# jerry102102102/RL_brain_trainer

Measured on AMD Instinct MI355X. Metric: env-steps/sec (whole node), Stage-5 Approach->Finisher PPO loops (rollout + update); value = the Approach loop, finisher.value = the Finisher loop, higher is better.
Workload: dtype f32

## Files before the change

### rl_brain_trainer_amd/csrc/kp1_mlp.hip

```cpp
#include <hip/hip_runtime.h>
#include <hip/hip_ext.h>

#include <cmath>
#include <cstddef>
#include <cstdlib>
#include <cstring>
#include <vector>

#include "../../include/kp1_ppo.h"
#include "kp1_device.hpp"
#include "kp1_host.hpp"

using kp1::fail;
using namespace kp1;

typedef float f32x16 __attribute__((ext_vector_type(16)));
typedef float f32x4 __attribute__((ext_vector_type(4)));

namespace {

constexpr int ACT = KP1_MLP_ACT, HEADS = 8;
constexpr float LOG_SQRT_2PI = 0.9189385332046727f;

enum { EPI_BIAS_TANH = 0, EPI_DTANH = 1 };
// ... 981 lines not shown

constexpr int ADAM_BLOCK = 256, VEC = 1;
template <bool POP = false>
__global__ void __launch_bounds__(ADAM_BLOCK) adam_kernel(float* __restrict__ p, float* __restrict__ g, float* __restrict__ m, float* __restrict__ v,
                                                   int64_t n, const double* __restrict__ partials, int n_partials, float lr, float eps, float max_norm,
                                                   float bc1, float bc2_sqrt, const ParamLayout L, const Packed k_, int zero_grad,
                                                   const int* __restrict__ step_counter, int host_step, const int* __restrict__ actor_extra,
                                                   unsigned r_partials, const float* __restrict__ hparams) {
  __shared__ float scale_s;
  const Packed k = POP ? packed_replica(k_, L, blockIdx.y) : k_;
  if constexpr (POP) {
    const unsigned o = blockIdx.y * (unsigned)n;
    p += o; g += o; m += o; v += o;
    partials += blockIdx.y * r_partials;
    if (hparams) {
      const float* e = hparams + blockIdx.y * (unsigned)HP_FIELDS;
      lr = e[HP_LR];
      eps = e[HP_EPS];
      max_norm = e[HP_MAX_NORM];
    }
  }
  const int64_t i0 = ((int64_t)blockIdx.x * ADAM_BLOCK + threadIdx.x) * VEC;
  float g_in[VEC], m_in[VEC], v_in[VEC], p_in[VEC];
#pragma unroll
  for (int j = 0; j < VEC; ++j) {
    const int64_t il = i0 + j < n ? i0 + j : n - 1;
    g_in[j] = g[il]; m_in[j] = m[il]; v_in[j] = v[il]; p_in[j] = p[il];
  }
  const int extra = *actor_extra;
  float base_step = (float)host_step;
  if (step_counter) base_step = (float)*step_counter;
  double s = 0.0;
  if (threadIdx.x < 64) {
    for (int q = threadIdx.x; q < n_partials; q += 64) s += partials[q];
    for (int off = 32; off > 0; off >>= 1) s += __shfl_xor(s, off);
  }
  if (threadIdx.x == 0) {
    const float norm = (float)sqrt(s);
    scale_s = max_norm > 0.f ? fminf(max_norm / (norm + 1e-6f), 1.f) : 1.f;
  }
  if (step_counter) {
    bc1 = 1.f - powf(0.9f, base_step);
    bc2_sqrt = sqrtf(1.f - powf(0.999f, base_step));
  }
  float bc1_a = bc1, bc2_sqrt_a = bc2_sqrt;
  if (extra != 0) {
    const float st = base_step + (float)extra;
    bc1_a = 1.f - powf(0.9f, st);
    bc2_sqrt_a = sqrtf(1.f - powf(0.999f, st));
  }
  __syncthreads();
  const float scale = scale_s;
  float pn[VEC], mn[VEC], vn[VEC];
#pragma unroll
  for (int j = 0; j < VEC; ++j) {
    const int64_t i = i0 + j;
    const bool actor = extra != 0 && ((i >= L.p_w1 && i < L.v_w1) || (i >= L.a_w && i < L.c_w));
    const float b1 = actor ? bc1_a : bc1, b2 = actor ? bc2_sqrt_a : bc2_sqrt;
    const float gi = g_in[j] * scale;
    mn[j] = 0.9f * m_in[j] + 0.1f * gi;
    vn[j] = 0.999f * v_in[j] + 0.001f * gi * gi;
    const float denom = sqrtf(vn[j]) / b2 + eps;
    pn[j] = p_in[j] - (lr / b1) * (mn[j] / denom);
  }
#pragma unroll
  for (int j = 0; j < VEC; ++j) {
    const int64_t i = i0 + j;
// ... 193 lines not shown
    const float pn = p_in - sh[1] * (mn / denom);
    m[i] = mn; v[i] = vn; p[i] = pn;
    pack_one(i, pn, L, k);
  }
}

__global__ void anchor_count_kernel(int* __restrict__ actor_extra) { *actor_extra += 1; }

#include "kp1_env_step.inc"
#include "kp1_eval_step.inc"
#include "kp1_mlp_tile.inc"
#include "kp1_mlp_fused.inc"

}

struct kp1_mlp {
  int device = 0, H = 0, Hp = 0, max_batch = 0;
  int K = 1;
  ParamLayout L;
  Packed k{};
  float* h1 = nullptr;
  float* h2 = nullptr;
  float* dz2 = nullptr;
  float* dz1 = nullptr;
  float* xf = nullptr;
  int bf16x3 = 0;
  unsigned short* sp_h1 = nullptr; unsigned short* sp_dz2 = nullptr; unsigned short* sp_dz1 = nullptr; unsigned short* sp_xf = nullptr;
  double* partials = nullptr;
  double* anchor_partials = nullptr;
  float* slab = nullptr;
  float* slab1 = nullptr;
  float* bslab = nullptr;
  float* hpart = nullptr;
  int n_finalize_blocks = 0;
  int* step_dev = nullptr;
  float* hparams_dev = nullptr;
  bool hparams_on = false;
  int last_s2_n = 0, last_s1_n = 0;
  int fused = 1;
  const float* last_params = nullptr;
  bool slab_stale = false;
  std::vector<void*> allocs;
  int profile = 0;
  struct ProfPair { hipEvent_t a, b; };
  std::vector<ProfPair> prof[KP1_MLP_PROFILE_SLOTS];
  int prof_used[KP1_MLP_PROFILE_SLOTS] = {0, 0, 0, 0};
};

namespace {
struct ProfSlotInFlight { hipEvent_t a = nullptr, b = nullptr; bool attached = false; };
thread_local ProfSlotInFlight tl_prof;

struct ProfScope {
  kp1_mlp* m; int slot; hipStream_t stream; bool on;
  ProfScope(kp1_mlp* m_, int slot_, hipStream_t s_) : m(m_), slot(slot_), stream(s_), on(m_->profile != 0) {
    if (!on) return;
    auto& v = m->prof[slot];
    if (m->prof_used[slot] >= (int)v.size()) {
      kp1_mlp::ProfPair p{};
      if (hipEventCreate(&p.a) != hipSuccess || hipEventCreate(&p.b) != hipSuccess) { on = false; return; }
      v.push_back(p);
    }
    tl_prof.a = v[m->prof_used[slot]].a;
    tl_prof.b = v[m->prof_used[slot]].b;
    tl_prof.attached = false;
  }
  ~ProfScope() {
    if (!on) return;
// ... 110 lines not shown
}

int launch_fused_infer_env(const FusedArgs& fa, int env_mode, hipStream_t stream) {
  const size_t bytes = sizeof(float) * FU_LDS_FLOATS;
  const dim3 grid((fa.n + FU_BM - 1) / FU_BM, 1, fa.value ? 2 : 1);
  if (env_mode == KP1_MODE_DOCK) {
    HIP_TRY(hipFuncSetAttribute((const void*)mlp_tile_kernel<false, 2, 2>, hipFuncAttributeMaxDynamicSharedMemorySize, (int)bytes));
    hipLaunchKernelGGL((mlp_tile_kernel<false, 2, 2>), grid, dim3(FU_NTH), bytes, stream, fa);
  } else {
    HIP_TRY(hipFuncSetAttribute((const void*)mlp_tile_kernel<false, 2, 1>, hipFuncAttributeMaxDynamicSharedMemorySize, (int)bytes));
    hipLaunchKernelGGL((mlp_tile_kernel<false, 2, 1>), grid, dim3(FU_NTH), bytes, stream, fa);
  }
  return KP1_OK;
}

int launch_fused_infer(const FusedArgs& fa, hipStream_t stream) {
  const size_t bytes = sizeof(float) * FU_LDS_FLOATS;
  const bool want_pi = fa.mean || fa.action || fa.clipped || fa.log_prob;
  if (!want_pi && !fa.value) return KP1_OK;
  FusedArgs f = fa;
  const bool both = want_pi && fa.value;
  if (!both) f.net_base = want_pi ? 0 : 1;
  const dim3 grid((fa.n + FU_BM - 1) / FU_BM, 1, both ? 2 : 1);
  if (fa.inp == 64) {
    HIP_TRY(hipFuncSetAttribute((const void*)mlp_tile_kernel<false, 2>, hipFuncAttributeMaxDynamicSharedMemorySize, (int)bytes));
    hipLaunchKernelGGL((mlp_tile_kernel<false, 2>), grid, dim3(FU_NTH), bytes, stream, f);
  } else {
    HIP_TRY(hipFuncSetAttribute((const void*)mlp_tile_kernel<false, 4>, hipFuncAttributeMaxDynamicSharedMemorySize, (int)bytes));
    hipLaunchKernelGGL((mlp_tile_kernel<false, 4>), grid, dim3(FU_NTH), bytes, stream, f);
  }
  return KP1_OK;
}

int launch_tn_frag(const TnFragArgs& t, hipStream_t stream) {
  if (t.n_chunks2 > 64 || t.n_chunks1 > 64) return fail(KP1_ERR_INVALID, "too many batch chunks for the partial-gradient slabs");
  const size_t bytes = sizeof(float) * TN_SPLIT_LDS_FLOATS;
  HIP_TRY(hipFuncSetAttribute((const void*)gemm_tn_split_kernel, hipFuncAttributeMaxDynamicSharedMemorySize, (int)bytes));
  KP1_LAUNCH(gemm_tn_split_kernel, dim3(32 * t.n_chunks2 + 16 * t.n_chunks1), dim3(256), bytes, stream, t);
  return KP1_OK;
}

int launch_forward_layers(kp1_mlp* m, const float* obs, int obs_stride, const int64_t* idx, int n, hipStream_t stream) {
  const int Hp = m->Hp, IN = m->L.IN, INP = m->L.INP;
  const int64_t act_stride = (int64_t)m->max_batch * Hp;
  GemmNT g{};
  g.reps = m->K;
  g.r_A = idx ? 0u : (unsigned)(n * obs_stride); g.r_gather = (unsigned)n;
  g.r_W = (unsigned)(2 * Hp * INP); g.r_bias = (unsigned)(2 * Hp); g.r_C = (unsigned)(2 * act_stride);
  g.A = obs; g.lda = obs_stride; g.strideA = 0; g.gather = idx;
  g.W = m->k.w1p; g.strideW = (int64_t)Hp * INP;
  g.bias = m->k.b1; g.strideBias = Hp;
  g.C = m->h1; g.ldc = Hp; g.strideC = act_stride;
  g.aux = nullptr; g.strideAux = 0; g.colsum = nullptr; g.strideColsum = 0;
  g.M = n; g.N = Hp; g.K = INP; g.Kreal = obs_stride >= INP ? INP : IN;
  int rc = launch_nt<EPI_BIAS_TANH>(g, stream);
  if (rc != KP1_OK) return rc;
  g.A = m->h1; g.lda = Hp; g.strideA = act_stride; g.gather = nullptr;
  g.r_A = (unsigned)(2 * act_stride); g.r_W = (unsigned)(2 * Hp * Hp);
  g.W = m->k.w2; g.strideW = (int64_t)Hp * Hp;
  g.bias = m->k.b2;
  g.C = m->h2;
  g.K = Hp; g.Kreal = Hp;
  rc = launch_nt<EPI_BIAS_TANH>(g, stream);
  if (rc != KP1_OK) return rc;
  HIP_TRY(kp1::launch_status());
  return KP1_OK;
}

}

namespace {
// ... 78 lines not shown
  m->H = hidden;
  m->L = make_layout(hidden, obs_dim);
  m->Hp = m->L.Hp;
  m->max_batch = (max_batch + 127) / 128 * 128;
  const int64_t Hp = m->Hp, mb = m->max_batch, INP = m->L.INP, K = m->K;
  auto alloc = [&](void** p, size_t bytes) -> int {
    if (hipMalloc(p, bytes) != hipSuccess) return fail(KP1_ERR_ALLOC, "hipMalloc failed in kp1_mlp_create");
    m->allocs.push_back(*p);
    return hipMemset(*p, 0, bytes) == hipSuccess ? KP1_OK : fail(KP1_ERR_NO_DEVICE, "hipMemset failed");
  };
  int rc = KP1_OK;
#define MLP_ALLOC(ptr, count) if (rc == KP1_OK) rc = alloc((void**)&(ptr), sizeof(*(ptr)) * (size_t)(count))
  MLP_ALLOC(m->k.w1p, K * 2 * Hp * INP);
  MLP_ALLOC(m->k.b1, K * 2 * Hp);
  MLP_ALLOC(m->k.w2, K * 2 * Hp * Hp);
  MLP_ALLOC(m->k.w2t, K * 2 * Hp * Hp);
  MLP_ALLOC(m->k.w1f, K * 2 * Hp * INP);
  MLP_ALLOC(m->k.w2f, K * 2 * Hp * Hp);
  MLP_ALLOC(m->k.w2tf, K * 2 * Hp * Hp);
  MLP_ALLOC(m->k.b2, K * 2 * Hp);
  MLP_ALLOC(m->k.w3, K * HEADS * Hp);
  MLP_ALLOC(m->k.b3, K * HEADS);
  MLP_ALLOC(m->k.log_std, K * HEADS);
  MLP_ALLOC(m->h1, K * 2 * mb * Hp);
  MLP_ALLOC(m->h2, K * 2 * mb * Hp);
  MLP_ALLOC(m->dz2, K * 2 * mb * Hp);
  MLP_ALLOC(m->dz1, K * 2 * mb * Hp);
  MLP_ALLOC(m->xf, mb * INP);
  MLP_ALLOC(m->partials, K * PARTIALS_STRIDE);
  if (Hp == 128) MLP_ALLOC(m->anchor_partials, K * ANCHOR_PARTIALS);
  MLP_ALLOC(m->slab, K * 64 * 2 * Hp * Hp);
  MLP_ALLOC(m->slab1, K * 64 * 2 * Hp * INP);
  MLP_ALLOC(m->step_dev, 4);
  if (K > 1) MLP_ALLOC(m->hparams_dev, K * HP_FIELDS);
  MLP_ALLOC(m->bslab, K * (mb / 32) * 2 * Hp);
  MLP_ALLOC(m->hpart, K * (mb / 32) * (10 * Hp + 32));
#undef MLP_ALLOC
  if (rc != KP1_OK) {
    kp1_mlp_destroy(m);
    return rc;
  }
  *out = m;
  return KP1_OK;
}
}

extern "C" {

int kp1_mlp_destroy(kp1_mlp* m) {
  if (!m) return KP1_OK;
  (void)hipSetDevice(m->device);
  (void)hipDeviceSynchronize();
  for (void* p : m->allocs) (void)hipFree(p);
  for (void* p : {(void*)m->sp_h1, (void*)m->sp_dz2, (void*)m->sp_dz1, (void*)m->sp_xf}) (void)hipFree(p);
  for (auto& v : m->prof)
    for (auto& pr : v) {
      (void)hipEventDestroy(pr.a);
      (void)hipEventDestroy(pr.b);
    }
  delete m;
  return KP1_OK;
}

int kp1_mlp_set_option(kp1_mlp* m, int32_t option, int32_t value) {
  if (!m) return fail(KP1_ERR_INVALID, "NULL argument");
  if (option == KP1_MLP_OPT_FUSED) {
// ... 249 lines not shown
    a.dz2 = m->dz2;
    a.hpart = m->hpart; a.hpart_stride = hpart_stride;
    a.r_act = (unsigned)(2 * act_stride); a.r_hpart = (unsigned)hpart_rep; a.r_partials = (unsigned)PARTIALS_STRIDE;
    a.hparams = pop && m->hparams_on ? m->hparams_dev : nullptr;
    {
      const dim3 hgrid((n + HEAD_ROWS - 1) / HEAD_ROWS, m->K);
      const size_t hbytes = sizeof(float) * (HEADS * Hp + HEAD_ROWS * 8 + 84 + 2 * HEAD_ROWS * (Hp + 4));
      if (pop) {
        HIP_TRY(hipFuncSetAttribute((const void*)head_train_kernel<128, true>, hipFuncAttributeMaxDynamicSharedMemorySize, (int)hbytes));
        hipLaunchKernelGGL((head_train_kernel<128, true>), hgrid, dim3(256), hbytes, stream, a);
      } else if (Hp == 256) {
        HIP_TRY(hipFuncSetAttribute((const void*)head_train_kernel<256>, hipFuncAttributeMaxDynamicSharedMemorySize, (int)hbytes));
        hipLaunchKernelGGL(head_train_kernel<256>, hgrid, dim3(256), hbytes, stream, a);
      } else {
        HIP_TRY(hipFuncSetAttribute((const void*)head_train_kernel<128>, hipFuncAttributeMaxDynamicSharedMemorySize, (int)hbytes));
        hipLaunchKernelGGL(head_train_kernel<128>, hgrid, dim3(256), hbytes, stream, a);
      }
    }
    GemmNT g{};
    g.A = m->dz2; g.lda = Hp; g.strideA = act_stride; g.gather = nullptr;
    g.W = m->k.w2t; g.strideW = (int64_t)Hp * Hp;
    g.bias = nullptr; g.strideBias = 0;
    g.C = m->dz1; g.ldc = Hp; g.strideC = act_stride;
    g.aux = m->h1; g.strideAux = act_stride;
    g.colsum = m->bslab; g.strideColsum = Hp;
    g.M = n; g.N = Hp; g.K = Hp; g.Kreal = Hp;
    g.reps = m->K;
    g.r_A = g.r_C = g.r_aux = (unsigned)(2 * act_stride); g.r_W = (unsigned)(2 * Hp * Hp);
    g.r_colsum = (unsigned)((m->max_batch / 32) * 2 * Hp);
    rc = launch_nt<EPI_DTANH>(g, stream);
    if (rc != KP1_OK) return rc;
  }

  int s2_n = 0, s1_n = 0;
  if (fused) {
    TnFragArgs t{};
    t.inp = INP;
    t.dz2 = m->dz2; t.h1 = m->h1; t.dz1 = m->dz1; t.act_stride = act_stride; t.xf = m->xf;
    t.slab2 = m->slab; t.s2_net = (int64_t)Hp * Hp; t.s2_chunk = 2 * t.s2_net;
    t.slab1 = m->slab1; t.s1_net = (int64_t)Hp * INP; t.s1_chunk = 2 * t.s1_net;
    t.groups = (n + FU_BM - 1) / FU_BM * (FU_BM / 8);
    auto up8 = [](int v) { return (v + 7) / 8 * 8; };
    t.cg2 = up8((t.groups + TN_SPLIT2 - 1) / TN_SPLIT2);
    t.cg1 = up8((t.groups + TN_SPLIT1 - 1) / TN_SPLIT1);
    t.n_chunks2 = (t.groups + t.cg2 - 1) / t.cg2;
    t.n_chunks1 = (t.groups + t.cg1 - 1) / t.cg1;
    if (m->bf16x3) {
      TnBf16Args b{};
      b.dz2 = m->sp_dz2; b.h1 = m->sp_h1; b.dz1 = m->sp_dz1; b.plane = (int64_t)2 * m->max_batch * Hp; b.net = (int64_t)m->max_batch * Hp;
      b.xf = m->sp_xf; b.plane_x = (int64_t)m->max_batch * INP; b.inp = INP;
      b.slab2 = t.slab2; b.s2_net = t.s2_net; b.s2_chunk = t.s2_chunk; b.slab1 = t.slab1; b.s1_net = t.s1_net; b.s1_chunk = t.s1_chunk;
      b.frags = t.groups / 2; b.cf2 = t.cg2 / 2; b.cf1 = t.cg1 / 2; b.n_chunks2 = t.n_chunks2; b.n_chunks1 = t.n_chunks1;
      const size_t bytes = sizeof(float) * TN_SPLIT_LDS_FLOATS;
      HIP_TRY(hipFuncSetAttribute((const void*)gemm_tn_bf16x3_kernel, hipFuncAttributeMaxDynamicSharedMemorySize, (int)bytes));
      ProfScope ps(m, KP1_MLP_PROFILE_WGRAD, stream);
      KP1_LAUNCH(gemm_tn_bf16x3_kernel, dim3(32 * b.n_chunks2 + 16 * b.n_chunks1), dim3(256), bytes, stream, b);
    } else {
      ProfScope ps(m, KP1_MLP_PROFILE_WGRAD, stream);
      rc = launch_tn_frag(t, stream);
    }
    if (rc != KP1_OK) return rc;
    s2_n = t.n_chunks2;
    s1_n = t.n_chunks1;
  } else {
    GemmTN t{};
    t.B = n;
    t.chunk = tn_chunk_rows(n, (Hp / 128) * (Hp / 128) * 2);
    t.D = m->dz2; t.ldd = Hp; t.strideD = act_stride;
    t.X = m->h1; t.ldx = Hp; t.strideX = act_stride; t.gatherX = nullptr;
    t.Nload = Hp; t.n_i_tiles = Hp / 128;
    rc = launch_tn(m, t, Hp / 128, Hp, m->slab, &s2_n, stream);
    if (rc != KP1_OK) return rc;
    t.D = m->dz1;
    t.X = obs; t.ldx = obs_stride; t.strideX = 0; t.gatherX = idx;
    t.Nload = obs_stride >= INP ? INP : IN; t.n_i_tiles = 1;
    t.chunk = tn_chunk_rows(n, (Hp / 128) * 2);
    rc = launch_tn(m, t, Hp / 128, INP, m->slab1, &s1_n, stream);
    if (rc != KP1_OK) return rc;
  }
  FinalizeArgs f{};
  f.L = L;
  f.slab2 = m->slab; f.s2_ld = Hp; f.s2_net = (int64_t)Hp * Hp; f.s2_chunk = 2 * f.s2_net; f.s2_n = s2_n;
  f.slab1 = m->slab1; f.s1_ld = INP; f.s1_net = (int64_t)Hp * INP; f.s1_chunk = 2 * f.s1_net; f.s1_n = s1_n;
  f.bslab = m->bslab; f.b_net = Hp; f.b_tile = 2 * Hp; f.b_n = fused ? (n + FU_BM - 1) / FU_BM * (FU_BM / 32) : nt_row_tiles(n, Hp);
  f.hpart = m->hpart; f.h_stride = 10 * Hp + 32; f.h_n = (n + HEAD_ROWS - 1) / HEAD_ROWS;
  f.ent_coef = ent_coef; f.inv_count = inv_count; f.log_std = m->k.log_std;
  f.grad = grad_out; f.stats = stats_out; f.sumsq = m->partials + 2 * N_PARTIALS;
  f.step_counter = m->step_dev;
  f.r_slab2 = (unsigned)(64 * f.s2_chunk); f.r_slab1 = (unsigned)(64 * f.s1_chunk); f.r_bslab = (unsigned)((m->max_batch / 32) * 2 * Hp);
  f.r_hpart = (unsigned)hpart_rep; f.r_sumsq = (unsigned)PARTIALS_STRIDE;
  f.hparams = pop && m->hparams_on ? m->hparams_dev : nullptr;
  const int n_main = (int)((finalize_vec_items(L) + 255) / 256);
  m->n_finalize_blocks = n_main + (int)((finalize_wide_count(L) + 3 + 31) / 32);
  if (m->n_finalize_blocks > 2048) return fail(KP1_ERR_INVALID, "parameter vector too large for the sum-of-squares partial buffer");
  {
    ProfScope ps(m, KP1_MLP_PROFILE_FINALIZE, stream);
    if (pop)
      KP1_LAUNCH(grad_finalize_kernel<true>, dim3(m->n_finalize_blocks, m->K), dim3(256), 0, stream, f, n_main);
    else
      KP1_LAUNCH(grad_finalize_kernel<false>, dim3(m->n_finalize_blocks), dim3(256), 0, stream, f, n_main);
  }
  HIP_TRY(kp1::launch_status());
  return KP1_OK;
}

int kp1_mlp_profile_read(kp1_mlp* m, float* out_us, int32_t* out_launches) {
  if (!m || !out_us || !out_launches) return fail(KP1_ERR_INVALID, "NULL argument to kp1_mlp_profile_read");
  int rc = mlp_check_device(m);
  if (rc != KP1_OK) return rc;
  for (int k = 0; k < KP1_MLP_PROFILE_SLOTS; ++k) {
    double total_ms = 0.0;
    for (int i = 0; i < m->prof_used[k]; ++i) {
      HIP_TRY(hipEventSynchronize(m->prof[k][i].b));
      float ms = 0.f;
      HIP_TRY(hipEventElapsedTime(&ms, m->prof[k][i].a, m->prof[k][i].b));
      total_ms += ms;
    }
    out_launches[k] = m->prof_used[k];
    out_us[k] = m->prof_used[k] > 0 ? (float)(total_ms * 1e3 / m->prof_used[k]) : 0.f;
    m->prof_used[k] = 0;
  }
  return KP1_OK;
}

int kp1_mlp_time_kernels(kp1_mlp* m, const float* obs, int32_t obs_stride, int32_t n, int32_t iters, float* out_ms, double* out_flops,
                         void* stream_) {
  if (!m || !obs || !out_ms || !out_flops || iters <= 0) return fail(KP1_ERR_INVALID, "bad argument to kp1_mlp_time_kernels");
  if (m->K > 1) return fail(KP1_ERR_UNSUPPORTED, "kp1_mlp_time_kernels is not available on population handles");
  if (n <= 0 || n > m->max_batch) return fail(KP1_ERR_INVALID, "n exceeds the workspace max_batch");
  int rc = mlp_check_device(m);
  if (rc != KP1_OK) return rc;
  hipStream_t stream = (hipStream_t)stream_;
  const int Hp = m->Hp, IN = m->L.IN, INP = m->L.INP;
// ... 9 lines not shown
    for (int it = 0; it < iters; ++it) {
      GemmNT g{};
      g.gather = nullptr; g.ldc = Hp; g.strideC = act_stride; g.M = n; g.N = Hp;
      if (which == 0) {
        g.A = m->h1; g.lda = Hp; g.strideA = act_stride; g.W = m->k.w2; g.strideW = (int64_t)Hp * Hp; g.bias = m->k.b2; g.strideBias = Hp;
        g.C = m->h2; g.K = Hp; g.Kreal = Hp;
        if (launch_nt<EPI_BIAS_TANH>(g, stream) != KP1_OK) return KP1_ERR_NO_DEVICE;
      } else if (which == 1) {
        g.A = m->dz2; g.lda = Hp; g.strideA = act_stride; g.W = m->k.w2t; g.strideW = (int64_t)Hp * Hp; g.C = m->dz1; g.aux = m->h1;
        g.strideAux = act_stride; g.K = Hp; g.Kreal = Hp;
        if (launch_nt<EPI_DTANH>(g, stream) != KP1_OK) return KP1_ERR_NO_DEVICE;
      } else if (which == 2) {
        GemmTN t{};
        t.B = n; t.chunk = tn_chunk_rows(n, (Hp / 128) * (Hp / 128) * 2);
        t.D = m->dz2; t.ldd = Hp; t.strideD = act_stride; t.X = m->h1; t.ldx = Hp; t.strideX = act_stride;
        t.Nload = Hp; t.n_i_tiles = Hp / 128;
        if (launch_tn(m, t, Hp / 128, Hp, m->slab, nullptr, stream) != KP1_OK) return KP1_ERR_NO_DEVICE;
      } else if (which == 3) {
        g.A = obs; g.lda = obs_stride; g.strideA = 0; g.W = m->k.w1p; g.strideW = (int64_t)Hp * INP; g.bias = m->k.b1; g.strideBias = Hp;
        g.C = m->h1; g.K = INP; g.Kreal = obs_stride >= INP ? INP : IN;
        if (launch_nt<EPI_BIAS_TANH>(g, stream) != KP1_OK) return KP1_ERR_NO_DEVICE;
      } else if (which == 4) {
        FusedArgs fa{};
        fa.obs = obs; fa.obs_stride = obs_stride; fa.Kreal = obs_stride >= INP ? INP : IN; fa.inp = INP; fa.idx = nullptr; fa.n = n;
        fa.k = m->k;
        fa.actions = m->h2; fa.old_logp = m->h2 + (int64_t)ACT * n; fa.adv = m->h2 + (int64_t)(ACT + 1) * n; fa.ret = m->h2 + (int64_t)(ACT + 2) * n;
        fa.adv_mode = 3; fa.adv_mean = 0.f; fa.adv_inv_std = 1.f;
        fa.clip_range = 0.2f; fa.vf_coef = 0.5f; fa.inv_count = 1.f / n;
        fa.h1 = m->h1; fa.dz2 = m->dz2; fa.dz1 = m->dz1; fa.act_stride = act_stride; fa.xf = m->xf;
        fa.bslab = m->bslab; fa.hpart = m->hpart; fa.hpart_stride = 10 * Hp + 32;
        if (launch_fused(fa, stream) != KP1_OK) return KP1_ERR_NO_DEVICE;
      } else {
        TnFragArgs t{};
    t.inp = INP;
        t.dz2 = m->dz2; t.h1 = m->h1; t.dz1 = m->dz1; t.act_stride = act_stride; t.xf = m->xf;
        t.slab2 = m->slab; t.s2_net = (int64_t)Hp * Hp; t.s2_chunk = 2 * t.s2_net;
        t.slab1 = m->slab1; t.s1_net = (int64_t)Hp * INP; t.s1_chunk = 2 * t.s1_net;
        t.groups = (n + FU_BM - 1) / FU_BM * (FU_BM / 8);
        t.cg2 = ((t.groups + TN_SPLIT2 - 1) / TN_SPLIT2 + 7) / 8 * 8;
        t.cg1 = ((t.groups + TN_SPLIT1 - 1) / TN_SPLIT1 + 7) / 8 * 8;
        t.n_chunks2 = (t.groups + t.cg2 - 1) / t.cg2;
        t.n_chunks1 = (t.groups + t.cg1 - 1) / t.cg1;
        if (launch_tn_frag(t, stream) != KP1_OK) return KP1_ERR_NO_DEVICE;
      }
    }
    HIP_TRY(hipEventRecord(e1, stream));
    HIP_TRY(hipEventSynchronize(e1));
    float ms = 0.f;
    HIP_TRY(hipEventElapsedTime(&ms, e0, e1));
    out_ms[which] = ms / iters;
    return KP1_OK;
  };
  for (int which : {3, 0, 1, 2}) {
    rc = time_it(which);
    if (rc != KP1_OK) return rc;
  }
  out_ms[4] = out_ms[5] = 0.f;
  out_flops[4] = out_flops[5] = 0.0;
  if (Hp == FU_HP) {
    for (int which : {4, 5}) {
      rc = time_it(which);
      if (rc != KP1_OK) return rc;
    }
  }
  const double M = n, H = Hp;
  out_flops[0] = 2.0 * 2.0 * M * H * H;
  out_flops[1] = 2.0 * 2.0 * M * H * H;
  out_flops[2] = 2.0 * 2.0 * M * H * H;
  out_flops[3] = 2.0 * 2.0 * M * H * INP;
  if (Hp == FU_HP) {
    out_flops[4] = 2.0 * 2.0 * M * (H * (double)INP + 2.0 * H * H);
    out_flops[5] = 2.0 * 2.0 * M * (H * H + H * (double)INP);
  }
  (void)hipEventDestroy(e0);
  (void)hipEventDestroy(e1);
  return KP1_OK;
// ... 53 lines not shown
    xcds += fresh ? 1 : 0;
  }
  out[0] = (int)total; out[1] = pairs; out[2] = same; out[3] = rr; out[4] = n_cus; out[5] = (int)seen.size(); out[6] = (int)host[total]; out[7] = xcds;
  return KP1_OK;
}

#ifdef KP1_CLK_TRACE
int kp1_debug_clk_trace(unsigned long long* out) {
  HIP_TRY(hipDeviceSynchronize());
  HIP_TRY(hipMemcpyFromSymbol(out, HIP_SYMBOL(kp1_clk_buf), sizeof(unsigned long long) * 2 * 1024 * 4));
  return KP1_OK;
}
#endif

#ifdef KP1_NT_TRACE
int kp1_debug_nt_trace(unsigned long long* out, int clear) {
  HIP_TRY(hipDeviceSynchronize());
  if (out) HIP_TRY(hipMemcpyFromSymbol(out, HIP_SYMBOL(kp1_nt_trace_buf), sizeof(unsigned long long) * KP1_TRACE_SLOTS * KP1_TRACE_WGS));
  if (clear) {
    std::vector<unsigned long long> z(KP1_TRACE_SLOTS * KP1_TRACE_WGS, 0ull);
    HIP_TRY(hipMemcpyToSymbol(HIP_SYMBOL(kp1_nt_trace_buf), z.data(), sizeof(unsigned long long) * z.size()));
  }
  return KP1_OK;
}
#endif

int kp1_mlp_adam_step(kp1_mlp* m, float* params, float* grad, float* exp_avg, float* exp_avg_sq, float lr, float eps, float max_grad_norm,
                      int32_t step, int32_t zero_grad, void* stream_) {
  if (!m || !params || !grad || !exp_avg || !exp_avg_sq) return fail(KP1_ERR_INVALID, "bad argument to kp1_mlp_adam_step");
  int rc = mlp_check_device(m);
  if (rc != KP1_OK) return rc;
  hipStream_t stream = (hipStream_t)stream_;
  const int64_t n = m->L.total;
  const bool fused_norm = (zero_grad & 2) && m->n_finalize_blocks > 0;
  const double* norm_partials = fused_norm ? m->partials + 2 * N_PARTIALS : m->partials + N_PARTIALS;
  const int n_norm_partials = fused_norm ? m->n_finalize_blocks : N_PARTIALS;
  ProfScope ps(m, KP1_MLP_PROFILE_ADAM, stream);
  const bool pop = m->K > 1;
  if (!fused_norm) {
    if (pop)
      hipLaunchKernelGGL(sumsq_partials_kernel<true>, dim3(N_PARTIALS, m->K), dim3(256), 0, stream, grad, n, m->partials + N_PARTIALS, (unsigned)PARTIALS_STRIDE);
    else
      hipLaunchKernelGGL(sumsq_partials_kernel<false>, dim3(N_PARTIALS), dim3(256), 0, stream, grad, n, m->partials + N_PARTIALS, 0u);
  }
  zero_grad = 0;
  const int host_step = step > 0 ? step : 1;
  const float bc1 = 1.f - std::pow(0.9f, (float)host_step);
  const float bc2 = 1.f - std::pow(0.999f, (float)host_step);
  Packed kfmt = m->k;
  const bool frag_only = m->fused && m->Hp == FU_HP;
  kfmt.formats = frag_only ? PACK_FRAG : (PACK_SLAB | PACK_FRAG);
  m->last_params = params;
  if (frag_only) m->slab_stale = true;
  const int* step_arg = step > 0 ? (const int*)nullptr : (const int*)m->step_dev;
  if (pop)
    KP1_LAUNCH(adam_kernel<true>, dim3((unsigned)((n + ADAM_BLOCK - 1) / ADAM_BLOCK), m->K), dim3(ADAM_BLOCK), 0, stream, params, grad, exp_avg, exp_avg_sq, n,
               norm_partials, n_norm_partials, lr, eps, max_grad_norm, bc1, std::sqrt(bc2), m->L, kfmt, zero_grad, step_arg, host_step,
               (const int*)m->step_dev + 1, (unsigned)PARTIALS_STRIDE, m->hparams_on ? (const float*)m->hparams_dev : (const float*)nullptr);
  else
    KP1_LAUNCH(adam_kernel<false>, dim3((unsigned)((n + ADAM_BLOCK - 1) / ADAM_BLOCK)), dim3(ADAM_BLOCK), 0, stream, params, grad, exp_avg, exp_avg_sq, n, norm_partials,
               n_norm_partials, lr, eps, max_grad_norm, bc1, std::sqrt(bc2), m->L, kfmt, zero_grad, step_arg, host_step, (const int*)m->step_dev + 1, 0u,
               (const float*)nullptr);
  HIP_TRY(kp1::launch_status());
  return KP1_OK;
}

int kp1_mlp_anchor_loss_grad(kp1_mlp* m, const float* obs, int32_t obs_stride, const int64_t* idx, int32_t n, const float* teacher_actions,
                             float loss_weight, float* grad_out, float* loss_out, void* stream_) {
  if (!m || !obs || !teacher_actions || !grad_out || !loss_out) return fail(KP1_ERR_INVALID, "NULL argument to kp1_mlp_anchor_loss_grad");
// ... 106 lines not shown
```

### rl_brain_trainer_amd/csrc/kp1_mlp_fused.inc

```

struct TnFragArgs {
  const float* dz2; const float* h1; const float* dz1; int64_t act_stride;
  const float* xf; int inp;
  float* slab2; int64_t s2_net, s2_chunk;
  float* slab1; int64_t s1_net, s1_chunk;
  int groups, cg2, n_chunks2, cg1, n_chunks1;
};

template <int RA, int CB>
__device__ __forceinline__ void tn_split_tile(const float* __restrict__ Af, int a_ncb, const float* __restrict__ Bf, int b_ncb, int g_begin, int g_end,
                                              float* __restrict__ out, int out_ld, float* lds) {
  constexpr int SG = 4;
  const int tid = threadIdx.x, lane = tid & 63, wave = __builtin_amdgcn_readfirstlane(tid >> 6);
  const int per = (max(g_end - g_begin, 0) + 3) >> 2;
  const int gb = min(g_begin + wave * per, g_end), ge = min(gb + per, g_end);
  const int64_t a_gs = (int64_t)a_ncb * 256, b_gs = (int64_t)b_ncb * 256;
  f32x4 ra[2][SG][RA], rb[2][SG][CB];
  f32x16 acc[RA][CB];
#pragma unroll
  for (int r = 0; r < RA; ++r)
#pragma unroll
    for (int c = 0; c < CB; ++c)
#pragma unroll
      for (int e = 0; e < 16; ++e) acc[r][c][e] = 0.f;
  KP1_TR(12)
  KP1_TR_HW(11)
  if (gb < ge) {
    const int g_last = ge - 1;
#define KP1_TNS_LOAD(set, g0)                                                                           \
  _Pragma("unroll") for (int u = 0; u < SG; ++u) {                                                      \
    const int gg_ = min((g0) + u, g_last);                                                              \
    _Pragma("unroll") for (int r = 0; r < RA; ++r) ra[set][u][r] = load16_sc1(Af, lane * 4 + gg_ * a_gs + r * 256); \
    _Pragma("unroll") for (int c = 0; c < CB; ++c) rb[set][u][c] = load16_sc1(Bf, lane * 4 + gg_ * b_gs + c * 256); \
  }
#define KP1_TNS_MFMA(set, g0)                                                                           \
  _Pragma("unroll") for (int u = 0; u < SG; ++u) {                                                      \
    const float keep_ = (g0) + u < ge ? 1.f : 0.f;                                                      \
    _Pragma("unroll") for (int i = 0; i < 4; ++i)                                                       \
      _Pragma("unroll") for (int r = 0; r < RA; ++r)                                                    \
        _Pragma("unroll") for (int c = 0; c < CB; ++c)                                                  \
          acc[r][c] = __builtin_amdgcn_mfma_f32_32x32x2f32(ra[set][u][r][i] * keep_, rb[set][u][c][i], acc[r][c], 0, 0, 0); \
  }
    KP1_TNS_LOAD(0, gb)
    for (int g = gb; g < ge; g += 2 * SG) {
// ... 2 lines not shown
      KP1_TNS_MFMA(0, g)
      __builtin_amdgcn_sched_barrier(0);
      KP1_TNS_LOAD(0, g + 2 * SG)
      __builtin_amdgcn_sched_barrier(0);
      KP1_TNS_MFMA(1, g + SG)
      __builtin_amdgcn_sched_barrier(0);
    }
#undef KP1_TNS_LOAD
#undef KP1_TNS_MFMA
  }
  KP1_TR(13)
  constexpr int TO = 32 * RA, TI = 32 * CB, LDP = TI + 8, Q = TI / 4;
  float* mine = lds + wave * (TO * LDP);
#pragma unroll
  for (int r = 0; r < RA; ++r)
#pragma unroll
    for (int c = 0; c < CB; ++c)
#pragma unroll
      for (int e = 0; e < 16; ++e) {
        const int o = r * 32 + (e & 3) + 8 * (e >> 2) + 4 * (lane >> 5);
        mine[o * LDP + c * 32 + (lane & 31)] = acc[r][c][e];
      }
  __syncthreads();
  KP1_TR(14)
#pragma unroll
  for (int j = 0; j < TO * Q / 256; ++j) {
    const int f = tid + 256 * j, o = f / Q, q = f % Q;
    const float* p0 = lds + o * LDP + 4 * q;
    const f32x4 v = ((*reinterpret_cast<const f32x4*>(p0) + *reinterpret_cast<const f32x4*>(p0 + TO * LDP)) +
                     *reinterpret_cast<const f32x4*>(p0 + 2 * TO * LDP)) + *reinterpret_cast<const f32x4*>(p0 + 3 * TO * LDP);
    store16_sc1(out, (int64_t)o * out_ld + 4 * q, v);
  }
  KP1_TR(15)
}
constexpr int TN_SPLIT_LDS_FLOATS = 4 * 64 * (64 + 8);

__global__ void __launch_bounds__(256, 2) gemm_tn_split_kernel(const TnFragArgs a) {
  extern __shared__ float lds[];
  KP1_CLK(1, 0)
  const int n2 = 32 * a.n_chunks2;
  if ((int)blockIdx.x < n2) {
    const int chunk = blockIdx.x % a.n_chunks2, tile = blockIdx.x / a.n_chunks2;
    const int net = tile >> 4, ot = (tile >> 2) & 3, it = tile & 3;
    const int g0 = chunk * a.cg2, g1 = min(g0 + a.cg2, a.groups);
    float* out = a.slab2 + chunk * a.s2_chunk + net * a.s2_net + (int64_t)(ot * 64) * FU_HP + it * 64;
    tn_split_tile<2, 2>(a.dz2 + net * a.act_stride + (ot * 2) * 256, 8, a.h1 + net * a.act_stride + (it * 2) * 256, 8, g0, g1, out, FU_HP, lds);
  } else {
    const int id = blockIdx.x - n2;
    const int chunk = id % a.n_chunks1, tile = id / a.n_chunks1;
    const int net = tile >> 3, ot = tile & 7;
    const int g0 = chunk * a.cg1, g1 = min(g0 + a.cg1, a.groups);
    const int inp = a.inp;
    float* out = a.slab1 + chunk * a.s1_chunk + net * a.s1_net + (int64_t)(ot * 32) * inp;
    if (inp == 64)
      tn_split_tile<1, 2>(a.dz1 + net * a.act_stride + ot * 256, 8, a.xf, 2, g0, g1, out, 64, lds);
    else
      tn_split_tile<1, 3>(a.dz1 + net * a.act_stride + ot * 256, 8, a.xf, 4, g0, g1, out, 128, lds);
  }
  KP1_CLK(1, 1)
}

struct TnBf16Args {
  const unsigned short* dz2; const unsigned short* h1; const unsigned short* dz1; int64_t plane, net;
  const unsigned short* xf; int64_t plane_x; int inp;
  float* slab2; int64_t s2_net, s2_chunk;
  float* slab1; int64_t s1_net, s1_chunk;
  int frags, cf2, n_chunks2, cf1, n_chunks1;
};

__device__ __forceinline__ bf16x8 tnb_load(const unsigned short* __restrict__ base, int64_t off) {
  const __amdgpu_buffer_rsrc_t r = __builtin_amdgcn_make_buffer_rsrc(const_cast<unsigned short*>(base), 0, 0x7fffffff, 0x00020000);
  return __builtin_bit_cast(bf16x8, __builtin_amdgcn_raw_buffer_load_b128(r, (int)(off * 2), 0, AUX_SC1));
}

template <int RA, int CB>
__device__ __forceinline__ void tn_bf16_tile(const unsigned short* __restrict__ Af, int64_t a_plane, int a_ncb, const unsigned short* __restrict__ Bf, int64_t b_plane,
                                             int b_ncb, int f_begin, int f_end, float* __restrict__ out, int out_ld, float* lds) {
  const int tid = threadIdx.x, lane = tid & 63, wave = __builtin_amdgcn_readfirstlane(tid >> 6);
  const int per = (max(f_end - f_begin, 0) + 3) >> 2;
  const int fb = min(f_begin + wave * per, f_end), fe = min(fb + per, f_end);
  const int64_t a_fs = (int64_t)a_ncb * 512, b_fs = (int64_t)b_ncb * 512;
  bf16x8 ra[2][3][RA], rb[2][3][CB];
  f32x16 acc[RA][CB];
#pragma unroll
  for (int r = 0; r < RA; ++r)
#pragma unroll
    for (int c = 0; c < CB; ++c)
#pragma unroll
      for (int e = 0; e < 16; ++e) acc[r][c][e] = 0.f;
  if (fb < fe) {
// ... 81 lines not shown
```

Before: 11.40 million.

## Fuse gradient finalize into weight-gradient split kernel via last-arriver reduction

The split-K weight-gradient kernel now reduces its own chunk partials. Each tile counts arriving chunk blocks with an atomic, and the last block sums the slabs, writes the final gradient and a per-tile sum of squares. Extra blocks handle the bias, head and log_std gradients that the separate finalize kernel used to produce, which removes one kernel launch and a pass over the slabs. The Adam norm reduction is also unrolled eight-wide. This adds atomic ordering risk and skips the finalize path only when the fused fp32 route runs.

```diff
diff --git a/rl_brain_trainer_amd/csrc/kp1_mlp.hip b/rl_brain_trainer_amd/csrc/kp1_mlp.hip
--- a/rl_brain_trainer_amd/csrc/kp1_mlp.hip
+++ b/rl_brain_trainer_amd/csrc/kp1_mlp.hip
@@ -1037,7 +1037,14 @@
   if (step_counter) base_step = (float)*step_counter;
   double s = 0.0;
   if (threadIdx.x < 64) {
-    for (int q = threadIdx.x; q < n_partials; q += 64) s += partials[q];
+    for (int q0 = threadIdx.x; q0 < n_partials; q0 += 64 * 8) {
+      double pv[8];
+#pragma unroll
+      for (int u = 0; u < 8; ++u) pv[u] = q0 + 64 * u < n_partials ? partials[q0 + 64 * u] : 0.0;
+#pragma unroll
+      for (int u = 0; u < 8; ++u)
+        if (q0 + 64 * u < n_partials) s += pv[u];
+    }
     for (int off = 32; off > 0; off >>= 1) s += __shfl_xor(s, off);
   }
   if (threadIdx.x == 0) {
@@ -1297,8 +1304,9 @@
   float* slab1 = nullptr;
   float* bslab = nullptr;
   float* hpart = nullptr;
-  int n_finalize_blocks = 0;
+  int n_norm_partials = 0;
   int* step_dev = nullptr;
+  unsigned* tn_arrivals = nullptr;
   float* hparams_dev = nullptr;
   bool hparams_on = false;
   int last_s2_n = 0, last_s1_n = 0;
@@ -1475,11 +1483,14 @@
   return KP1_OK;
 }
 
-int launch_tn_frag(const TnFragArgs& t, hipStream_t stream) {
-  if (t.n_chunks2 > 64 || t.n_chunks1 > 64) return fail(KP1_ERR_INVALID, "too many batch chunks for the partial-gradient slabs");
+int launch_tn_frag(const TnFragArgs& t, const FinalizeArgs& f, int wide_blocks, hipStream_t stream) {
+  static_assert(TN_SPLIT2 == TN_MAX_CHUNKS2 && TN_SPLIT1 == TN_MAX_CHUNKS1, "the reducer holds one register set per batch chunk");
+  if (t.n_chunks2 < 1 || t.n_chunks2 > TN_MAX_CHUNKS2 || t.n_chunks1 < 1 || t.n_chunks1 > TN_MAX_CHUNKS1)
+    return fail(KP1_ERR_INVALID, "batch chunk count outside what the weight-gradient reducer holds");
+  if (!t.arrivals || !f.grad || !f.sumsq) return fail(KP1_ERR_INVALID, "NULL argument to the weight-gradient launch");
   const size_t bytes = sizeof(float) * TN_SPLIT_LDS_FLOATS;
   HIP_TRY(hipFuncSetAttribute((const void*)gemm_tn_split_kernel, hipFuncAttributeMaxDynamicSharedMemorySize, (int)bytes));
-  KP1_LAUNCH(gemm_tn_split_kernel, dim3(32 * t.n_chunks2 + 16 * t.n_chunks1), dim3(256), bytes, stream, t);
+  KP1_LAUNCH(gemm_tn_split_kernel, dim3(TN_TILES2 * t.n_chunks2 + TN_TILES1 * t.n_chunks1 + wide_blocks), dim3(256), bytes, stream, t, f);
   return KP1_OK;
 }
 
@@ -1624,6 +1635,7 @@
   MLP_ALLOC(m->slab, K * 64 * 2 * Hp * Hp);
   MLP_ALLOC(m->slab1, K * 64 * 2 * Hp * INP);
   MLP_ALLOC(m->step_dev, 4);
+  MLP_ALLOC(m->tn_arrivals, 64);
   if (K > 1) MLP_ALLOC(m->hparams_dev, K * HP_FIELDS);
   MLP_ALLOC(m->bslab, K * (mb / 32) * 2 * Hp);
   MLP_ALLOC(m->hpart, K * (mb / 32) * (10 * Hp + 32));
@@ -1939,6 +1951,18 @@
     if (rc != KP1_OK) return rc;
   }
 
+  FinalizeArgs f{};
+  f.L = L;
+  f.slab2 = m->slab; f.s2_ld = Hp; f.s2_net = (int64_t)Hp * Hp; f.s2_chunk = 2 * f.s2_net; f.s2_n = 0;
+  f.slab1 = m->slab1; f.s1_ld = INP; f.s1_net = (int64_t)Hp * INP; f.s1_chunk = 2 * f.s1_net; f.s1_n = 0;
+  f.bslab = m->bslab; f.b_net = Hp; f.b_tile = 2 * Hp; f.b_n = fused ? (n + FU_BM - 1) / FU_BM * (FU_BM / 32) : nt_row_tiles(n, Hp);
+  f.hpart = m->hpart; f.h_stride = 10 * Hp + 32; f.h_n = (n + HEAD_ROWS - 1) / HEAD_ROWS;
+  f.ent_coef = ent_coef; f.inv_count = inv_count; f.log_std = m->k.log_std;
+  f.grad = grad_out; f.stats = stats_out; f.sumsq = m->partials + 2 * N_PARTIALS;
+  f.step_counter = m->step_dev;
+  f.r_slab2 = (unsigned)(64 * f.s2_chunk); f.r_slab1 = (unsigned)(64 * f.s1_chunk); f.r_bslab = (unsigned)((m->max_batch / 32) * 2 * Hp);
+  f.r_hpart = (unsigned)hpart_rep; f.r_sumsq = (unsigned)PARTIALS_STRIDE;
+  f.hparams = pop && m->hparams_on ? m->hparams_dev : nullptr;
   int s2_n = 0, s1_n = 0;
   if (fused) {
     TnFragArgs t{};
@@ -1963,8 +1987,17 @@
       ProfScope ps(m, KP1_MLP_PROFILE_WGRAD, stream);
       KP1_LAUNCH(gemm_tn_bf16x3_kernel, dim3(32 * b.n_chunks2 + 16 * b.n_chunks1), dim3(256), bytes, stream, b);
     } else {
-      ProfScope ps(m, KP1_MLP_PROFILE_WGRAD, stream);
-      rc = launch_tn_frag(t, stream);
+      const int wide_blocks = (int)((finalize_wide_count(L) + 3 + 31) / 32);
+      t.arrivals = m->tn_arrivals;
+      m->n_norm_partials = TN_TILES2 + TN_TILES1 + wide_blocks;
+      if (m->n_norm_partials > 2048) return fail(KP1_ERR_INVALID, "parameter vector too large for the sum-of-squares partial buffer");
+      {
+        ProfScope ps(m, KP1_MLP_PROFILE_WGRAD, stream);
+        rc = launch_tn_frag(t, f, wide_blocks, stream);
+      }
+      if (rc != KP1_OK) return rc;
+      HIP_TRY(kp1::launch_status());
+      return KP1_OK;
     }
     if (rc != KP1_OK) return rc;
     s2_n = t.n_chunks2;
@@ -1985,27 +2018,16 @@
     rc = launch_tn(m, t, Hp / 128, INP, m->slab1, &s1_n, stream);
     if (rc != KP1_OK) return rc;
   }
-  FinalizeArgs f{};
-  f.L = L;
-  f.slab2 = m->slab; f.s2_ld = Hp; f.s2_net = (int64_t)Hp * Hp; f.s2_chunk = 2 * f.s2_net; f.s2_n = s2_n;
-  f.slab1 = m->slab1; f.s1_ld = INP; f.s1_net = (int64_t)Hp * INP; f.s1_chunk = 2 * f.s1_net; f.s1_n = s1_n;
-  f.bslab = m->bslab; f.b_net = Hp; f.b_tile = 2 * Hp; f.b_n = fused ? (n + FU_BM - 1) / FU_BM * (FU_BM / 32) : nt_row_tiles(n, Hp);
-  f.hpart = m->hpart; f.h_stride = 10 * Hp + 32; f.h_n = (n + HEAD_ROWS - 1) / HEAD_ROWS;
-  f.ent_coef = ent_coef; f.inv_count = inv_count; f.log_std = m->k.log_std;
-  f.grad = grad_out; f.stats = stats_out; f.sumsq = m->partials + 2 * N_PARTIALS;
-  f.step_counter = m->step_dev;
-  f.r_slab2 = (unsigned)(64 * f.s2_chunk); f.r_slab1 = (unsigned)(64 * f.s1_chunk); f.r_bslab = (unsigned)((m->max_batch / 32) * 2 * Hp);
-  f.r_hpart = (unsigned)hpart_rep; f.r_sumsq = (unsigned)PARTIALS_STRIDE;
-  f.hparams = pop && m->hparams_on ? m->hparams_dev : nullptr;
+  f.s2_n = s2_n; f.s1_n = s1_n;
   const int n_main = (int)((finalize_vec_items(L) + 255) / 256);
-  m->n_finalize_blocks = n_main + (int)((finalize_wide_count(L) + 3 + 31) / 32);
-  if (m->n_finalize_blocks > 2048) return fail(KP1_ERR_INVALID, "parameter vector too large for the sum-of-squares partial buffer");
+  m->n_norm_partials = n_main + (int)((finalize_wide_count(L) + 3 + 31) / 32);
+  if (m->n_norm_partials > 2048) return fail(KP1_ERR_INVALID, "parameter vector too large for the sum-of-squares partial buffer");
   {
     ProfScope ps(m, KP1_MLP_PROFILE_FINALIZE, stream);
     if (pop)
-      KP1_LAUNCH(grad_finalize_kernel<true>, dim3(m->n_finalize_blocks, m->K), dim3(256), 0, stream, f, n_main);
+      KP1_LAUNCH(grad_finalize_kernel<true>, dim3(m->n_norm_partials, m->K), dim3(256), 0, stream, f, n_main);
     else
-      KP1_LAUNCH(grad_finalize_kernel<false>, dim3(m->n_finalize_blocks), dim3(256), 0, stream, f, n_main);
+      KP1_LAUNCH(grad_finalize_kernel<false>, dim3(m->n_norm_partials), dim3(256), 0, stream, f, n_main);
   }
   HIP_TRY(kp1::launch_status());
   return KP1_OK;
@@ -2081,7 +2103,7 @@
         if (launch_fused(fa, stream) != KP1_OK) return KP1_ERR_NO_DEVICE;
       } else {
         TnFragArgs t{};
-    t.inp = INP;
+        t.inp = INP;
         t.dz2 = m->dz2; t.h1 = m->h1; t.dz1 = m->dz1; t.act_stride = act_stride; t.xf = m->xf;
         t.slab2 = m->slab; t.s2_net = (int64_t)Hp * Hp; t.s2_chunk = 2 * t.s2_net;
         t.slab1 = m->slab1; t.s1_net = (int64_t)Hp * INP; t.s1_chunk = 2 * t.s1_net;
@@ -2090,7 +2112,13 @@
         t.cg1 = ((t.groups + TN_SPLIT1 - 1) / TN_SPLIT1 + 7) / 8 * 8;
         t.n_chunks2 = (t.groups + t.cg2 - 1) / t.cg2;
         t.n_chunks1 = (t.groups + t.cg1 - 1) / t.cg1;
-        if (launch_tn_frag(t, stream) != KP1_OK) return KP1_ERR_NO_DEVICE;
+        t.arrivals = m->tn_arrivals;
+        FinalizeArgs f{};
+        f.L = m->L;
+        f.grad = m->slab + 32 * t.s2_chunk;
+        f.sumsq = m->partials + 2 * N_PARTIALS;
+        m->n_norm_partials = 0;
+        if (launch_tn_frag(t, f, 0, stream) != KP1_OK) return KP1_ERR_NO_DEVICE;
       }
     }
     HIP_TRY(hipEventRecord(e1, stream));
@@ -2210,9 +2238,9 @@
   if (rc != KP1_OK) return rc;
   hipStream_t stream = (hipStream_t)stream_;
   const int64_t n = m->L.total;
-  const bool fused_norm = (zero_grad & 2) && m->n_finalize_blocks > 0;
+  const bool fused_norm = (zero_grad & 2) && m->n_norm_partials > 0;
   const double* norm_partials = fused_norm ? m->partials + 2 * N_PARTIALS : m->partials + N_PARTIALS;
-  const int n_norm_partials = fused_norm ? m->n_finalize_blocks : N_PARTIALS;
+  const int n_norm_partials = fused_norm ? m->n_norm_partials : N_PARTIALS;
   ProfScope ps(m, KP1_MLP_PROFILE_ADAM, stream);
   const bool pop = m->K > 1;
   if (!fused_norm) {
diff --git a/rl_brain_trainer_amd/csrc/kp1_mlp_fused.inc b/rl_brain_trainer_amd/csrc/kp1_mlp_fused.inc
--- a/rl_brain_trainer_amd/csrc/kp1_mlp_fused.inc
+++ b/rl_brain_trainer_amd/csrc/kp1_mlp_fused.inc
@@ -5,11 +5,16 @@
   float* slab2; int64_t s2_net, s2_chunk;
   float* slab1; int64_t s1_net, s1_chunk;
   int groups, cg2, n_chunks2, cg1, n_chunks1;
+  unsigned* arrivals;
 };
-
-template <int RA, int CB>
+constexpr int TN_TILES2 = 32, TN_TILES1 = 16;
+constexpr int TN_MAX_CHUNKS2 = 8, TN_MAX_CHUNKS1 = 16;
+
+template <int RA, int CB, int NC>
 __device__ __forceinline__ void tn_split_tile(const float* __restrict__ Af, int a_ncb, const float* __restrict__ Bf, int b_ncb, int g_begin, int g_end,
-                                              float* __restrict__ out, int out_ld, float* lds) {
+                                              float* __restrict__ slab0, int64_t chunk_stride, int chunk, int n_chunks, int out_ld, float* lds,
+                                              unsigned* arrival, float* __restrict__ gdst, int g_ld, int g_cols, double* __restrict__ sumsq) {
+  float* __restrict__ out = slab0 + chunk * chunk_stride;
   constexpr int SG = 4;
   const int tid = threadIdx.x, lane = tid & 63, wave = __builtin_amdgcn_readfirstlane(tid >> 6);
   const int per = (max(g_end - g_begin, 0) + 3) >> 2;
@@ -78,30 +83,167 @@
     store16_sc1(out, (int64_t)o * out_ld + 4 * q, v);
   }
   KP1_TR(15)
+  asm volatile("s_waitcnt vmcnt(0)" ::: "memory");
+  __syncthreads();
+  if (tid == 0) reinterpret_cast<unsigned*>(lds)[0] = __hip_atomic_fetch_add(arrival, 1u, __ATOMIC_RELAXED, __HIP_MEMORY_SCOPE_AGENT);
+  __syncthreads();
+  const unsigned ticket = __builtin_amdgcn_readfirstlane(reinterpret_cast<const unsigned*>(lds)[0]);
+  if (ticket == (unsigned)(n_chunks - 1)) {
+    __builtin_amdgcn_fence(__ATOMIC_ACQUIRE, "wavefront");
+    constexpr int J = TO * Q / 256;
+    f32x4 part[J][NC];
+#pragma unroll
+    for (int j = 0; j < J; ++j) {
+      const int f = tid + 256 * j, o = f / Q, q = f % Q;
+#pragma unroll
+      for (int c = 0; c < NC; ++c) part[j][c] = load16_sc1(slab0, min(c, n_chunks - 1) * chunk_stride + (int64_t)o * out_ld + 4 * q);
+    }
+    double gsq = 0.0;
+#pragma unroll
+    for (int j = 0; j < J; ++j) {
+      const int f = tid + 256 * j, o = f / Q, q = f % Q;
+      f32x4 s = {0.f, 0.f, 0.f, 0.f};
+#pragma unroll
+      for (int c = 0; c < NC; ++c)
+        if (c < n_chunks) s += part[j][c];
+      if (4 * q < g_cols) {
+        float* d = gdst + (int64_t)o * g_ld + 4 * q;
+#pragma unroll
+        for (int e = 0; e < 4; ++e) {
+          d[e] = s[e];
+          gsq += (double)s[e] * (double)s[e];
+        }
+      }
+    }
+    for (int off = 32; off > 0; off >>= 1) gsq += __shfl_xor(gsq, off);
+    double* sq = reinterpret_cast<double*>(lds) + 1;
+    if (lane == 0) sq[wave] = gsq;
+    __syncthreads();
+    if (tid == 0) {
+      *sumsq = ((sq[0] + sq[1]) + sq[2]) + sq[3];
+      __hip_atomic_store(arrival, 0u, __ATOMIC_RELAXED, __HIP_MEMORY_SCOPE_AGENT);
+    }
+  }
 }
 constexpr int TN_SPLIT_LDS_FLOATS = 4 * 64 * (64 + 8);
 
-__global__ void __launch_bounds__(256, 2) gemm_tn_split_kernel(const TnFragArgs a) {
+__device__ __forceinline__ void tn_wide_block(const FinalizeArgs& a, unsigned wb, float* lds) {
+  const ParamLayout& L = a.L;
+  const unsigned tid = threadIdx.x, el = tid & 31, strand = tid >> 5;
+  const unsigned H = (unsigned)L.H, Hp = (unsigned)L.Hp;
+  const unsigned n_heads = (unsigned)(L.total - L.a_w), n_wide = ACT + 4 * H + n_heads;
+  const unsigned e = wb * 32 + el;
+  const bool is_grad = e < n_wide, is_stat = !is_grad && e < n_wide + 3;
+  const float* p = a.hpart;
+  unsigned stride = (unsigned)a.h_stride;
+  int n = a.h_n;
+  float add = 0.f;
+  int64_t flat = 0;
+  if (is_grad) {
+    if (e < (unsigned)ACT) {
+      flat = L.log_std + e;
+      p = a.hpart + 10 * Hp + 8 + e;
+      add = -a.ent_coef;
+    } else if (e < ACT + 4 * H) {
+      const unsigned k = e - ACT, which = k / H, r = k - which * H;
+      if (which & 1) {
+        flat = (which == 1 ? L.p_b2 : L.v_b2) + r;
+        p = a.hpart + (which == 1 ? 8 : 9) * Hp + r;
+      } else {
+        flat = (which == 0 ? L.p_b1 : L.v_b1) + r;
+        p = a.bslab + (which == 0 ? 0 : a.b_net) + r;
+        stride = (unsigned)a.b_tile; n = a.b_n;
+      }
+    } else {
+      const unsigned k = e - (ACT + 4 * H);
+      flat = L.a_w + k;
+      if (k < ACT * H) {
+        const unsigned row = k / H;
+        p = a.hpart + row * Hp + (k - row * H);
+      } else if (k < ACT * H + ACT) {
+        p = a.hpart + 10 * Hp + (k - ACT * H);
+      } else if (k < ACT * H + ACT + H) {
+        p = a.hpart + 7 * Hp + (k - ACT * H - ACT);
+      } else {
+        p = a.hpart + 10 * Hp + 7;
+      }
+    }
+  } else if (is_stat) {
+    p = a.hpart + 10 * Hp + 15 + (e - n_wide);
+  }
+  float part = 0.f;
+  if (is_grad || is_stat) {
+    int c = (int)strand;
+    for (; c + 8 * 31 < n; c += 8 * 32) {
+      float v[32];
+#pragma unroll
+      for (int u = 0; u < 32; ++u) v[u] = p[(size_t)((unsigned)(c + 8 * u) * stride)];
+#pragma unroll
+      for (int u = 0; u < 32; ++u) part += v[u];
+    }
+    for (; c < n; c += 8) part += p[(size_t)((unsigned)c * stride)];
+  }
+  float* red = lds;
+  red[strand * 32 + el] = part;
+  __syncthreads();
+  float gval = 0.f;
+  if (tid < 32) {
+    float t = red[el];
+#pragma unroll
+    for (int k = 1; k < 8; ++k) t += red[k * 32 + el];
+    if (is_grad) {
+      gval = t + add;
+      a.grad[flat] = gval;
+    } else if (is_stat && a.stats) {
+      const unsigned k = e - n_wide;
+      a.stats[k == 2 ? 3 : k] += t * a.inv_count;
+    }
+  }
+  if (wb == 0 && tid == 64 && a.step_counter) *a.step_counter += 1;
+  if (wb == 0 && tid == 65 && a.stats) {
+    float ent = 0.f;
+    for (int k = 0; k < ACT; ++k) ent += 0.5f + LOG_SQRT_2PI + a.log_std[k];
+    a.stats[2] += ent;
+  }
+  double w = (double)gval * (double)gval;
+  for (int off = 32; off > 0; off >>= 1) w += __shfl_xor(w, off);
+  double* sq = reinterpret_cast<double*>(lds + 256);
+  if ((tid & 63) == 0) sq[tid >> 6] = w;
+  __syncthreads();
+  if (tid == 0) a.sumsq[TN_TILES2 + TN_TILES1 + wb] = ((sq[0] + sq[1]) + sq[2]) + sq[3];
+}
+
+__global__ void __launch_bounds__(256, 2) gemm_tn_split_kernel(const TnFragArgs a, const FinalizeArgs f) {
   extern __shared__ float lds[];
   KP1_CLK(1, 0)
-  const int n2 = 32 * a.n_chunks2;
+  const int n2 = TN_TILES2 * a.n_chunks2, n1 = TN_TILES1 * a.n_chunks1;
+  const ParamLayout& L = f.L;
   if ((int)blockIdx.x < n2) {
     const int chunk = blockIdx.x % a.n_chunks2, tile = blockIdx.x / a.n_chunks2;
     const int net = tile >> 4, ot = (tile >> 2) & 3, it = tile & 3;
     const int g0 = chunk * a.cg2, g1 = min(g0 + a.cg2, a.groups);
-    float* out = a.slab2 + chunk * a.s2_chunk + net * a.s2_net + (int64_t)(ot * 64) * FU_HP + it * 64;
-    tn_split_tile<2, 2>(a.dz2 + net * a.act_stride + (ot * 2) * 256, 8, a.h1 + net * a.act_stride + (it * 2) * 256, 8, g0, g1, out, FU_HP, lds);
-  } else {
+    float* slab0 = a.slab2 + net * a.s2_net + (int64_t)(ot * 64) * FU_HP + it * 64;
+    float* gdst = f.grad + (net ? L.v_w2 : L.p_w2) + (int64_t)(ot * 64) * FU_HP + it * 64;
+    tn_split_tile<2, 2, TN_MAX_CHUNKS2>(a.dz2 + net * a.act_stride + (ot * 2) * 256, 8, a.h1 + net * a.act_stride + (it * 2) * 256, 8, g0, g1, slab0, a.s2_chunk,
+                                        chunk, a.n_chunks2, FU_HP, lds, a.arrivals + tile, gdst, FU_HP, 64, f.sumsq + tile);
+  } else if ((int)blockIdx.x < n2 + n1) {
     const int id = blockIdx.x - n2;
     const int chunk = id % a.n_chunks1, tile = id / a.n_chunks1;
     const int net = tile >> 3, ot = tile & 7;
     const int g0 = chunk * a.cg1, g1 = min(g0 + a.cg1, a.groups);
     const int inp = a.inp;
-    float* out = a.slab1 + chunk * a.s1_chunk + net * a.s1_net + (int64_t)(ot * 32) * inp;
+    float* slab0 = a.slab1 + net * a.s1_net + (int64_t)(ot * 32) * inp;
+    float* gdst = f.grad + (net ? L.v_w1 : L.p_w1) + (int64_t)(ot * 32) * L.IN;
+    unsigned* arrival = a.arrivals + TN_TILES2 + tile;
+    double* sumsq = f.sumsq + TN_TILES2 + tile;
     if (inp == 64)
-      tn_split_tile<1, 2>(a.dz1 + net * a.act_stride + ot * 256, 8, a.xf, 2, g0, g1, out, 64, lds);
+      tn_split_tile<1, 2, TN_MAX_CHUNKS1>(a.dz1 + net * a.act_stride + ot * 256, 8, a.xf, 2, g0, g1, slab0, a.s1_chunk, chunk, a.n_chunks1, 64, lds, arrival, gdst,
+                                          L.IN, L.IN, sumsq);
     else
-      tn_split_tile<1, 3>(a.dz1 + net * a.act_stride + ot * 256, 8, a.xf, 4, g0, g1, out, 128, lds);
+      tn_split_tile<1, 3, TN_MAX_CHUNKS1>(a.dz1 + net * a.act_stride + ot * 256, 8, a.xf, 4, g0, g1, slab0, a.s1_chunk, chunk, a.n_chunks1, 128, lds, arrival, gdst,
+                                          L.IN, L.IN, sumsq);
+  } else {
+    tn_wide_block(f, blockIdx.x - (unsigned)(n2 + n1), lds);
   }
   KP1_CLK(1, 1)
 }
```

Result: no change. 11.37 million (-0.3%).
